# fpthink/3D-WSIS

Measured on AMD Instinct MI355X. Metric: scenes/sec fwd+bwd ScanNet 2cm (~150k voxels) @1/8 GPU; HBM GB/s vs roofline, higher is better.
Workload: dtype f32; 1 GPU; C2: 1 synthetic ScanNet-shaped scene on 1 GPU, 2 cm voxels, fwd+bwd+AdamW step (SubMConv3d UNet 32..160 + ECC GNN + edge affinity + MultiTaskLoss); per-batch segment CSRs / edge graph and all rulebooks are rebuilt inside every step; active_voxels=153685, points=199790, superpoints=2289, edges=20054, scenes_per_gpu=1, global_batch=1, parallelism=scene-sharded dp1

## Files before the change

### 3d-wsis_amd/csrc/loss.hip

```cpp
#include <cstdlib>

#include "common.h"

namespace wsis {
namespace {

constexpr int LOSS_CMAX = 32;
static_assert(LOSS_CMAX == 32, "the error texts of the host checks say 32");
constexpr int SL_THREADS = 256;
constexpr int SL_VALS = 3 * LOSS_CMAX + 2;
constexpr int SL_TP = SL_THREADS + 4;
constexpr int SL_MAX_BLOCKS = 512;

struct SoftmaxRow {
  float v[LOSS_CMAX];
  __device__ __forceinline__ void load(const float* __restrict__ row, int C) {
#pragma unroll
    for (int c = 0; c < LOSS_CMAX; ++c) v[c] = row[c < C ? c : C - 1];
#pragma unroll
    for (int c = 0; c < LOSS_CMAX; ++c) v[c] = c < C ? v[c] : -INFINITY;
  }
  __device__ __forceinline__ float exp_sum(int C, float& Z) {
    float m = v[0];
#pragma unroll
// ... 14 lines not shown
#pragma unroll
  for (int q = 0; q < NV; ++q) {
    double v = (double)a[q];
#pragma unroll
    for (int off = 32; off >= 1; off >>= 1) v += __shfl_xor(v, off, 64);
    if (lane == 0) sh[wave * NV + q] = v;
  }
  __syncthreads();
}
template <int NV, int NW>
__device__ __forceinline__ double block_sum_read(const double* sh, int q) {
  double t = 0.0;
  for (int w = 0; w < NW; ++w) t += sh[w * NV + q];
  return t;
}

__global__ __launch_bounds__(SL_THREADS) void sem_loss_fwd_kernel(const float* __restrict__ x,
                                                                  const int64_t* __restrict__ y, int64_t N, int C,
                                                                  int64_t ignore, float* __restrict__ partial) {
  extern __shared__ __attribute__((aligned(16))) float sl_tile[];
  float A[LOSS_CMAX], B[LOSS_CMAX], K[LOSS_CMAX];
#pragma unroll
  for (int c = 0; c < LOSS_CMAX; ++c) A[c] = B[c] = K[c] = 0.0f;
  float ce = 0.0f, n = 0.0f;
  for (int64_t r = blockIdx.x * (int64_t)blockDim.x + threadIdx.x; r < N; r += (int64_t)gridDim.x * blockDim.x) {
    const int64_t lab = y[r];
    if (lab == ignore) continue;
    SoftmaxRow s;
    s.load(x + r * C, C);
    float xl = 0.0f, Z;
#pragma unroll
    for (int c = 0; c < LOSS_CMAX; ++c)
      if ((int64_t)c == lab && c < C) xl = s.v[c];
    const float m = s.exp_sum(C, Z);
    const float inv = 1.0f / Z, logZ = logf(Z);
#pragma unroll
    for (int c = 0; c < LOSS_CMAX; ++c) {
      const float p = s.v[c] * inv;
      const bool hit = (int64_t)c == lab;
      B[c] += p * p;
      A[c] += hit ? p : 0.0f;
      K[c] += hit ? 1.0f : 0.0f;
    }
    ce += (m + logZ) - xl;
    n += 1.0f;
  }
#pragma unroll
  for (int c = 0; c < LOSS_CMAX; ++c) {
    sl_tile[c * SL_TP + threadIdx.x] = A[c];
    sl_tile[(LOSS_CMAX + c) * SL_TP + threadIdx.x] = B[c];
    sl_tile[(2 * LOSS_CMAX + c) * SL_TP + threadIdx.x] = K[c];
  }
  sl_tile[(3 * LOSS_CMAX) * SL_TP + threadIdx.x] = ce;
  sl_tile[(3 * LOSS_CMAX + 1) * SL_TP + threadIdx.x] = n;
  __syncthreads();
  if (threadIdx.x < SL_VALS) {
    const float4* row = reinterpret_cast<const float4*>(sl_tile + threadIdx.x * SL_TP);
    float s = 0.0f;
#pragma unroll 8
    for (int q = 0; q < SL_THREADS / 4; ++q) {
      const float4 v = row[q];
      s += v.x;
      s += v.y;
      s += v.z;
      s += v.w;
    }
    partial[(int64_t)blockIdx.x * SL_VALS + threadIdx.x] = s;
  }
}

__global__ __launch_bounds__(1024) void sem_loss_final_kernel(const float* __restrict__ partial, int nblk, int C,
                                                              float* __restrict__ out, float* __restrict__ saved) {
  __shared__ double sums[128];
  __shared__ double psub[8][128];
  const int v = threadIdx.x & 127, sub = threadIdx.x >> 7;
  double s = 0.0;
  if (v < SL_VALS)
    for (int b = sub; b < nblk; b += 64) {
      float t[8];
#pragma unroll
      for (int j = 0; j < 8; ++j) {
        const int bb = b + 8 * j;
        t[j] = bb < nblk ? partial[(int64_t)bb * SL_VALS + v] : 0.0f;
      }
#pragma unroll
      for (int j = 0; j < 8; ++j) s += (double)t[j];
    }
  psub[sub][v] = s;
  __syncthreads();
  if (sub == 0)
    sums[v] = ((psub[0][v] + psub[1][v]) + (psub[2][v] + psub[3][v])) + ((psub[4][v] + psub[5][v]) + (psub[6][v] + psub[7][v]));
  __syncthreads();
  if (threadIdx.x == 0) {
    const double eps = 1e-5;
    const double n = sums[3 * LOSS_CMAX + 1];
    double dice_sum = 0.0;
    for (int c = 0; c < C; ++c) {
      const double num = 2.0 * sums[c] + eps;
      const double den = sums[LOSS_CMAX + c] + sums[2 * LOSS_CMAX + c] + 1e-4 + eps;
      saved[c] = (float)num;
      saved[C + c] = (float)den;
      dice_sum += 1.0 - num / den;
    }
    saved[2 * C] = (float)n;
    out[0] = (float)(sums[3 * LOSS_CMAX] / n + dice_sum / (double)C);
    out[1] = (float)n;
  }
}

__global__ __launch_bounds__(SL_THREADS) void sem_loss_bwd_kernel(const float* __restrict__ x,
                                                                  const int64_t* __restrict__ y, int64_t N, int C,
                                                                  int64_t ignore, const float* __restrict__ saved,
                                                                  const float* __restrict__ gout,
                                                                  float* __restrict__ dx) {
  __shared__ float s_num[LOSS_CMAX], s_den[LOSS_CMAX];
  if (threadIdx.x < LOSS_CMAX) {
    s_num[threadIdx.x] = threadIdx.x < C ? saved[threadIdx.x] : 0.0f;
    s_den[threadIdx.x] = threadIdx.x < C ? saved[C + threadIdx.x] : 1.0f;
  }
  __syncthreads();
  const float g = gout[0];
  const float inv_n = 1.0f / saved[2 * C];
  const float inv_c = 1.0f / (float)C;
  __shared__ float tile[SL_THREADS * (LOSS_CMAX + 1)];
  const int pitch = C | 1;
  for (int64_t r0 = blockIdx.x * (int64_t)blockDim.x; r0 < N; r0 += (int64_t)gridDim.x * blockDim.x) {
    const int64_t r = r0 + threadIdx.x;
    float* const mine = tile + threadIdx.x * pitch;
    const int64_t lab = r < N ? y[r] : ignore;
    if (lab == ignore) {
      for (int c = 0; c < C; ++c) mine[c] = 0.0f;
    } else {
      SoftmaxRow s;
      float Z;
      s.load(x + r * C, C);
      s.exp_sum(C, Z);
      const float inv = 1.0f / Z;
      float gp[LOSS_CMAX];
      float dot = 0.0f;
#pragma unroll
      for (int c = 0; c < LOSS_CMAX; ++c) {
        const float p = s.v[c] * inv;
        s.v[c] = p;
        const float den = s_den[c];
        gp[c] = c < C ? inv_c * (2.0f * p * s_num[c] / (den * den) - (((int64_t)c == lab) ? 2.0f / den : 0.0f)) : 0.0f;
        dot += gp[c] * p;
      }
#pragma unroll
      for (int c = 0; c < LOSS_CMAX; ++c)
        if (c < C) mine[c] = g * (s.v[c] * (gp[c] - dot) + (s.v[c] - (((int64_t)c == lab) ? 1.0f : 0.0f)) * inv_n);
    }
    __syncthreads();
    const int64_t rows = N - r0 < (int64_t)blockDim.x ? N - r0 : (int64_t)blockDim.x;
    float* const dst = dx + r0 * C;
    for (int64_t f = threadIdx.x; f < rows * C; f += blockDim.x) {
      const int rr = (int)(f / C), cc = (int)(f - (int64_t)rr * C);
      dst[f] = tile[rr * pitch + cc];
    }
    __syncthreads();
  }
}

constexpr int SR_THREADS = 1024;

struct RegRow {
  float p[3], g[3], np, ip, ig;
  static __device__ __forceinline__ bool dropped(const int64_t* __restrict__ sem, const int64_t* __restrict__ ins,
                                                 int64_t r, int64_t ignore) {
    return sem[r] == ignore || ins[r] == ignore;
  }
  __device__ __forceinline__ void load(const float* __restrict__ p_off, const float* __restrict__ g_off, int64_t r) {
    float pp = 0.f, gg = 0.f;
// ... 187 lines not shown
    const int t = threadIdx.x + u * DL_THREADS;
    v[u] = src[t < n ? t : 0];
  }
}
template <int NU, typename T>
__device__ __forceinline__ void dl_store(const T (&v)[NU], int n, T* dst) {
#pragma unroll
  for (int u = 0; u < NU; ++u) {
    const int t = threadIdx.x + u * DL_THREADS;
    if (t < n) dst[t] = v[u];
  }
}

__device__ __forceinline__ void dl_stage(const float* __restrict__ x, const int64_t* __restrict__ ins,
                                         const int64_t* __restrict__ sem, int S, int I, int64_t ignore, float* xs,
                                         short* slot) {
  constexpr int NR = DL_ROWS / DL_THREADS;
  float v[NR * DL_D];
  int64_t a[NR], b[NR];
  dl_load(x, S * DL_D, v);
  dl_load(ins, S, a);
  dl_load(sem, S, b);
  dl_store(v, S * DL_D, xs);
#pragma unroll
  for (int u = 0; u < NR; ++u) {
    const int r = threadIdx.x + u * DL_THREADS;
    if (r < S) slot[r] = (a[u] != ignore && b[u] != ignore && a[u] >= 0 && a[u] < I) ? (short)a[u] : (short)-1;
  }
}

template <typename On, typename Term>
__device__ __forceinline__ float dl_slot_sums(const short* slot, float* psum, int S, int I, On on, Term term) {
  const int nch = dl_chunks(I), per = I * 8;
  if (threadIdx.x < nch * per) {
    const int ch = threadIdx.x / per, u = threadIdx.x - ch * per;
    const int a = u >> 3, d = u & 7;
    const int r0 = (int)((int64_t)S * ch / nch), r1 = (int)((int64_t)S * (ch + 1) / nch);
    float s = 0.f;
    if (on(a, d)) {
      for (int r = r0; r < r1; r += 8) {
        short sl[8];
        float v[8];
// ... 24 lines not shown
  return fmaxf(2.0f * delta_d - l1, 0.f);
}

__device__ __forceinline__ float dl_mu_norm(const float (*mu)[8], int a) {
  float t2 = 0.f;
#pragma unroll
  for (int d = 0; d < DL_D; ++d) t2 += mu[a][d] * mu[a][d];
  return sqrtf(t2);
}

template <typename T>
__device__ __forceinline__ T dl_pair_den(T n) {
  return n * (n - T(1)) > T(1) ? n * (n - T(1)) : T(1);
}

__global__ __launch_bounds__(DL_THREADS) void disc_loss_fwd_kernel(const float* __restrict__ x,
                                                                   const int64_t* __restrict__ ins,
                                                                   const int64_t* __restrict__ sem, int S, int I,
                                                                   int64_t ignore, DlParams P, float* __restrict__ out,
                                                                   float* __restrict__ saved) {
  __shared__ float xs[DL_ROWS * DL_D];
  __shared__ short slot[DL_ROWS];
  __shared__ float mu[DL_SLOTS][8];
  __shared__ float psum[DL_THREADS];
  __shared__ double red[DL_THREADS / 64];
  dl_stage(x, ins, sem, S, I, ignore, xs, slot);
  __syncthreads();
  const float sum = dl_slot_sums(slot, psum, S, I, [](int, int) { return true; },
                                 [&](int, int d, int r) { return d < DL_D ? xs[r * DL_D + d] : 1.0f; });
  if (threadIdx.x < I * 8) mu[threadIdx.x >> 3][threadIdx.x & 7] = sum;
  __syncthreads();
  {
    const bool act = threadIdx.x < I * 8;
    const int a = threadIdx.x >> 3, d = threadIdx.x & 7;
    const float c = act ? mu[a][7] : 1.0f, sv = act ? mu[a][d] : 0.0f;
    __syncthreads();
    if (act && d < DL_D) mu[a][d] = sv / fmaxf(c, 1.0f);
  }
  __syncthreads();
  double lvar = 0.0, ldist = 0.0, lreg = 0.0, n = 0.0;
  float* kk = saved + DL_SLOTS * 8;
  for (int r = threadIdx.x; r < S; r += DL_THREADS) {
    const int a = slot[r];
    float k = 0.f;
    if (a >= 0) {
      float t2 = 0.f;
#pragma unroll
      for (int d = 0; d < DL_D; ++d) {
        const float e = xs[r * DL_D + d] - mu[a][d];
        t2 += e * e;
      }
      const float t = sqrtf(t2), h = fmaxf(t - P.delta_v, 0.f);
      lvar += (double)(h * h / mu[a][7]);
      k = t > 0.f ? 2.0f * h / t : 0.f;
    }
    kk[r] = k;
  }
  for (int q = threadIdx.x; q < I * I; q += DL_THREADS) {
    const int a = q / I, b = q - a * I;
    if (a != b && mu[a][7] > 0.f && mu[b][7] > 0.f) {
      const float h = dl_pair_hinge(mu, a, b, P.delta_d);
      ldist += (double)(h * h);
    }
  }
  if (threadIdx.x < I && mu[threadIdx.x][7] > 0.f) {
    lreg = (double)dl_mu_norm(mu, threadIdx.x);
    n = 1.0;
  }
  auto total = [&](double v) {
    const double one[1] = {v};
    __syncthreads();
    block_sum_stage(one, red);
    return block_sum_read<1, DL_THREADS / 64>(red, 0);
  };
  lvar = total(lvar), ldist = total(ldist), lreg = total(lreg), n = total(n);
  for (int t = threadIdx.x; t < DL_SLOTS * 8; t += DL_THREADS) saved[t] = (t >> 3) < I ? mu[t >> 3][t & 7] : 0.f;
  if (threadIdx.x == 0) {
    out[0] = (float)(P.p_var * (lvar / n) + P.p_dist * (ldist / dl_pair_den(n)) + P.p_reg * lreg);
    saved[DL_SLOTS * 8 + DL_ROWS] = (float)n;
  }
}

__global__ __launch_bounds__(DL_THREADS) void disc_loss_bwd_kernel(const float* __restrict__ x,
                                                                   const int64_t* __restrict__ ins,
                                                                   const int64_t* __restrict__ sem, int S, int I,
                                                                   int64_t ignore, DlParams P,
                                                                   const float* __restrict__ saved,
                                                                   const float* __restrict__ gout,
                                                                   float* __restrict__ dx) {
  __shared__ float xs[DL_ROWS * DL_D];
  __shared__ short slot[DL_ROWS];
  __shared__ float mu[DL_SLOTS][8];
  __shared__ float gmu[DL_SLOTS][8];
  __shared__ float psum[DL_THREADS];
  __shared__ float kk[DL_ROWS];
  dl_stage(x, ins, sem, S, I, ignore, xs, slot);
  for (int t = threadIdx.x; t < DL_SLOTS * 8; t += DL_THREADS) mu[t >> 3][t & 7] = saved[t];
  {
    float kv[DL_ROWS / DL_THREADS];
    dl_load(saved + DL_SLOTS * 8, S, kv);
    dl_store(kv, S, kk);
  }
  __syncthreads();
  const float n = saved[DL_SLOTS * 8 + DL_ROWS];
  const float den = dl_pair_den(n);
  const float via = dl_slot_sums(slot, psum, S, I, [&](int a, int d) { return d < DL_D && mu[a][7] > 0.f; },
                                 [&](int a, int d, int r) { return kk[r] * (xs[r * DL_D + d] - mu[a][d]); });
  if (threadIdx.x < I * 8) {
    const int a = threadIdx.x >> 3, d = threadIdx.x & 7;
    float gsum = 0.f;
    const float c = mu[a][7];
    if (d < DL_D && c > 0.f) {
      for (int b = 0; b < I; ++b) {
        if (b == a || !(mu[b][7] > 0.f)) continue;
        const float h = dl_pair_hinge(mu, a, b, P.delta_d);
        const float df = mu[a][d] - mu[b][d];
        const float sg = df > 0.f ? 1.f : (df < 0.f ? -1.f : 0.f);
        gsum += (P.p_dist / den) * 4.0f * h * (-sg);
      }
      const float nm = dl_mu_norm(mu, a);
      if (nm > 0.f) gsum += P.p_reg * mu[a][d] / nm;
      gsum += -(P.p_var / (n * c)) * via;
    }
    gmu[a][d] = gsum;
  }
  __syncthreads();
  const float g = gout[0];
  for (int t = threadIdx.x; t < S * DL_D; t += DL_THREADS) {
    const int r = t / DL_D, d = t - r * DL_D;
    const int a = slot[r];
    float v = 0.f;
    if (a >= 0) {
      const float c = mu[a][7];
      v = g * ((P.p_var / (n * c)) * kk[r] * (xs[t] - mu[a][d]) + gmu[a][d] / c);
    }
    dx[t] = v;
  }
}

const char* disc_loss_bad_args(const float* x, const int64_t* ins, const int64_t* sem, int64_t S, int32_t D,
                               int32_t n_slots, const float* saved) {
  if (!(S >= 1 && S <= DL_ROWS && D == DL_D && n_slots >= 1 && n_slots <= DL_SLOTS))
    return "1 <= rows <= 4096, 7 features, 1 <= slots <= 64";
  return x && ins && sem && saved ? nullptr : "null pointer";
}

int sl_blocks(int64_t N) {
  const char* e = tune_env("WSIS_SL_BLOCKS");
  int cap = e ? atoi(e) : 256;
  if (cap < 1 || cap > SL_MAX_BLOCKS) cap = SL_MAX_BLOCKS;
  int64_t b = ceil_div(N > 0 ? N : 1, SL_THREADS);
  if (b > cap) b = cap;
  return (int)b;
}

}
}

using namespace wsis;
// ... 8 lines not shown
int wsis_semantic_loss_fwd(const float* d_scores, const int64_t* d_labels, int64_t N, int32_t C, int64_t ignore_label,
                           float* d_out2, float* d_saved, void* d_ws, int64_t ws_bytes, void* stream) {
  WSIS_REQUIRE(N >= 0 && C >= 1 && C <= LOSS_CMAX, "1 <= classes <= 32");
  WSIS_REQUIRE(d_out2 && d_saved && d_ws, "null pointer");
  WSIS_REQUIRE(N == 0 || (d_scores && d_labels), "null input");
  WSIS_REQUIRE(ws_bytes >= wsis_semantic_loss_workspace_bytes(N), "workspace too small");
  hipStream_t st = as_stream(stream);
  const int nblk = sl_blocks(N);
  float* partial = static_cast<float*>(d_ws);
  const size_t ldsb = (size_t)SL_VALS * SL_TP * sizeof(float);
  static bool attr_set = false;
  if (!attr_set) {
    WSIS_HIP_CHECK(hipFuncSetAttribute((const void*)sem_loss_fwd_kernel, hipFuncAttributeMaxDynamicSharedMemorySize, (int)ldsb));
    attr_set = true;
  }
  hipLaunchKernelGGL(sem_loss_fwd_kernel, dim3(nblk), dim3(SL_THREADS), ldsb, st, d_scores, d_labels, N, (int)C,
                     ignore_label, partial);
  WSIS_LAUNCH_CHECK();
  hipLaunchKernelGGL(sem_loss_final_kernel, dim3(1), dim3(1024), 0, st, partial, nblk, (int)C, d_out2, d_saved);
  WSIS_LAUNCH_CHECK();
  return WSIS_OK;
}

int wsis_semantic_loss_bwd(const float* d_scores, const int64_t* d_labels, int64_t N, int32_t C, int64_t ignore_label,
                           const float* d_saved, const float* d_grad_loss, float* d_dscores, void* stream) {
  WSIS_REQUIRE(N >= 0 && C >= 1 && C <= LOSS_CMAX, "1 <= classes <= 32");
  if (N == 0) return WSIS_OK;
  WSIS_REQUIRE(d_scores && d_labels && d_saved && d_grad_loss && d_dscores, "null pointer");
  hipLaunchKernelGGL(sem_loss_bwd_kernel, dim3(grid_for(N, SL_THREADS)), dim3(SL_THREADS), 0, as_stream(stream),
                     d_scores, d_labels, N, (int)C, ignore_label, d_saved, d_grad_loss, d_dscores);
  WSIS_LAUNCH_CHECK();
  return WSIS_OK;
}

int wsis_sp_regression_loss_fwd(const float* d_pred_off, const float* d_gt_off, const float* d_pred_occ,
                                const float* d_gt_occ, const float* d_pred_size, const float* d_gt_size,
                                const int64_t* d_sem_label, const int64_t* d_ins_label, int64_t S,
                                int64_t ignore_label, float* d_out5, void* stream) {
  WSIS_REQUIRE(S >= 0 && d_out5, "bad args");
  WSIS_REQUIRE(S == 0 || (d_pred_off && d_gt_off && d_pred_occ && d_gt_occ && d_pred_size && d_gt_size &&
                          d_sem_label && d_ins_label), "null pointer");
  hipLaunchKernelGGL(sp_reg_fwd_kernel, dim3(1), dim3(SR_THREADS), 0, as_stream(stream), d_pred_off, d_gt_off,
                     d_pred_occ, d_gt_occ, d_pred_size, d_gt_size, d_sem_label, d_ins_label, S, ignore_label, d_out5);
  WSIS_LAUNCH_CHECK();
  return WSIS_OK;
// ... 56 lines not shown
  hipLaunchKernelGGL(loss_sum_kernel, dim3(1), dim3(1), 0, as_stream(stream), t[0], t[1], t[2], t[3], t[4], t[5], t[6], t[7], (int)n,
                     (unsigned)paired, d_out);
  WSIS_LAUNCH_CHECK();
  return WSIS_OK;
}

int32_t wsis_disc_loss_saved_floats(void) { return DL_SLOTS * 8 + DL_ROWS + 1; }

int wsis_disc_loss_fwd(const float* d_x, const int64_t* d_ins_label, const int64_t* d_sem_label, int64_t S,
                       int32_t D, int32_t n_slots, int64_t ignore_label, float delta_v, float delta_d, float p_var,
                       float p_dist, float p_reg, float* d_out1, float* d_saved, void* stream) {
  const char* bad = disc_loss_bad_args(d_x, d_ins_label, d_sem_label, S, D, n_slots, d_saved);
  WSIS_REQUIRE(!bad, bad);
  WSIS_REQUIRE(d_out1, "null pointer");
  const DlParams P = {delta_v, delta_d, p_var, p_dist, p_reg};
  hipLaunchKernelGGL(disc_loss_fwd_kernel, dim3(1), dim3(DL_THREADS), 0, as_stream(stream), d_x, d_ins_label,
                     d_sem_label, (int)S, (int)n_slots, ignore_label, P, d_out1, d_saved);
  WSIS_LAUNCH_CHECK();
  return WSIS_OK;
}

int wsis_disc_loss_bwd(const float* d_x, const int64_t* d_ins_label, const int64_t* d_sem_label, int64_t S,
                       int32_t D, int32_t n_slots, int64_t ignore_label, float delta_v, float delta_d, float p_var,
                       float p_dist, float p_reg, const float* d_saved, const float* d_grad_loss, float* d_dx,
                       void* stream) {
  const char* bad = disc_loss_bad_args(d_x, d_ins_label, d_sem_label, S, D, n_slots, d_saved);
  WSIS_REQUIRE(!bad, bad);
  WSIS_REQUIRE(d_grad_loss && d_dx, "null pointer");
  const DlParams P = {delta_v, delta_d, p_var, p_dist, p_reg};
  hipLaunchKernelGGL(disc_loss_bwd_kernel, dim3(1), dim3(DL_THREADS), 0, as_stream(stream), d_x, d_ins_label,
                     d_sem_label, (int)S, (int)n_slots, ignore_label, P, d_saved, d_grad_loss, d_dx);
  WSIS_LAUNCH_CHECK();
  return WSIS_OK;
}

}
```

### 3d-wsis_amd/model/losses_3D_WSIS.py

```python
import functools
import os

import torch
import torch.nn as nn
import torch.nn.functional as F


class _NullLogger(object):
    def info(self, *a, **k):
        pass


def _ops():
    import wsis_ops
    return wsis_ops


def _on(switch, default="1"):
    return os.environ.get(switch, default) != "0"


class MultiTaskLoss(nn.Module):
    def __init__(self, logger, param_loss, param_model):
        super().__init__()
# ... 126 lines not shown
    def _sp_discriminative(self, inp, indexed, valid, loss_out):
        feats, sp_batch_offsets = inp["sp_discriminative_features"]
        sp_sem_labels, sp_ins_labels = inp["superpoint_labels"]
        offs = [int(o) for o in sp_batch_offsets]
        slots = inp.get("sp_instance_slots")
        d_losses = []
        for i in range(1, len(offs)):
            b, e = offs[i - 1], offs[i]
            n_slots = int(slots[i - 1]) if slots is not None else 0
            ins = sp_ins_labels[b:e]
            if indexed:
                keep = valid()[0][b:e]
                d_loss, _, _, _ = self.discriminative_loss(feats[b:e][keep], ins[keep])
            elif (feats.is_cuda and self.discriminative_feature_dim == 7 and _on("WSIS_FUSE_DISC_LOSS")
                  and 1 <= n_slots <= _ops().DISC_MAX_SLOTS and 1 <= e - b <= _ops().DISC_MAX_ROWS):
                d_loss = _ops().discriminative_loss(feats[b:e], ins, sp_sem_labels[b:e], n_slots, self.ignore_label,
                                                    self.delta_v, self.delta_d, self.param_var, self.param_dist,
                                                    self.param_reg)
            elif 1 <= n_slots <= 512:
                d_loss = self.discriminative_loss_slots(feats[b:e], ins, valid()[0][b:e], n_slots)
            else:
                d_loss = self.discriminative_loss_masked(feats[b:e], ins, valid()[0][b:e])
            d_losses.append(d_loss.view(-1))
        sp_d_loss = torch.mean(torch.cat(d_losses)) if len(d_losses) != 1 else d_losses[0].reshape(())
        loss_out["superpoint_discriminative_loss"] = (sp_d_loss, feats.shape[0])
        return sp_d_loss

    def _sum_terms(self, terms, paired):
        for name, t in terms:
            self._log(name, t)
        terms = [t for _, t in terms]
# ... 98 lines not shown
```

### 3d-wsis_amd/wsis_ops.py

```python
import ctypes
import os

import numpy as np
import torch
from torch.autograd import Function

import wsis_native as _n
from torch_scatter import SegmentCSR


def branch_stream(device, i=0):
    if os.environ.get("WSIS_BRANCH", "1") == "0" or device.type != "cuda":
        return None
    from spconv import ops as sp_ops
    return sp_ops._side_stream(device)


class EdgeGraph(object):

    def __init__(self, edge_u, edge_v, num_nodes, num_src=None, csr_u=None, csr_v=None):
        _n.require_cuda(edge_u, edge_v)
        self.eu = edge_u.contiguous().long()
        self.ev = edge_v.contiguous().long()
        self.E = self.eu.numel()
# ... 835 lines not shown
        lib = _n.hip()
        scores = scores.contiguous().float()
        labels = labels.contiguous().long()
        N, C = scores.shape
        out = torch.empty(2, dtype=torch.float32, device=scores.device)
        saved = torch.empty(2 * C + 1, dtype=torch.float32, device=scores.device)
        ws_bytes = lib.wsis_semantic_loss_workspace_bytes(N)
        ws = torch.empty(ws_bytes, dtype=torch.uint8, device=scores.device)
        _n.check(lib.wsis_semantic_loss_fwd(_n.ptr(scores), _n.ptr(labels), N, C, int(ignore_label), _n.ptr(out),
                                            _n.ptr(saved), _n.ptr(ws), ws_bytes, _n.stream_ptr()),
                 "semantic_loss_fwd")
        ctx.save_for_backward(scores, labels, saved)
        ctx.ignore_label = int(ignore_label)
        loss, n_valid = out[0], out[1]
        ctx.mark_non_differentiable(n_valid)
        return loss, n_valid

    @staticmethod
    def backward(ctx, g_loss, _g_n):
        scores, labels, saved = ctx.saved_tensors
        N, C = scores.shape
        d = torch.empty_like(scores)
        g = g_loss.contiguous().float()
        _n.check(_n.hip().wsis_semantic_loss_bwd(_n.ptr(scores), _n.ptr(labels), N, C, ctx.ignore_label,
                                                 _n.ptr(saved), _n.ptr(g), _n.ptr(d), _n.stream_ptr()),
                 "semantic_loss_bwd")
        return d, None, None


def semantic_point_loss(scores, labels, ignore_label=-100):
    return _SemanticPointLoss.apply(scores, labels, ignore_label)


class _SpCrossEntropy(Function):

# ... 1 lines not shown
    def forward(ctx, scores, labels, ignore_label):
        _n.require_cuda(scores, labels)
        scores = scores.contiguous().float()
        labels = labels.contiguous().long()
        S, C = scores.shape
        out = torch.empty(3, dtype=torch.float32, device=scores.device)
        lib = _n.hip()
        ws_bytes = lib.wsis_sp_ce_loss_workspace_bytes(S)
        ws = torch.empty(ws_bytes, dtype=torch.uint8, device=scores.device)
        _n.check(lib.wsis_sp_ce_loss_fwd(_n.ptr(scores), _n.ptr(labels), S, C, int(ignore_label), _n.ptr(out), _n.ptr(ws),
                                         ws_bytes, _n.ptr(_n.sync_block(scores.device)), _n.stream_ptr()), "sp_ce_loss_fwd")
        ctx.save_for_backward(scores, labels, out)
        ctx.ignore_label = int(ignore_label)
        loss, total = out[0], out[1]
        ctx.mark_non_differentiable(total)
        return loss, total

    @staticmethod
    def backward(ctx, g_loss, _g_total):
        scores, labels, out = ctx.saved_tensors
        S, C = scores.shape
        d = torch.empty_like(scores)
        _n.check(_n.hip().wsis_sp_ce_loss_bwd(_n.ptr(scores), _n.ptr(labels), S, C, ctx.ignore_label, _n.ptr(out),
                                              _n.ptr(g_loss.contiguous().float()), _n.ptr(d), _n.stream_ptr()),
                 "sp_ce_loss_bwd")
        return d, None, None


def superpoint_cross_entropy(scores, labels, ignore_label=-100):
    return _SpCrossEntropy.apply(scores, labels, ignore_label)


class _LossSum(Function):

    @staticmethod
# ... 24 lines not shown
        pred_off, gt_off, pred_occ, gt_occ, pred_size, gt_size = (f(pred_off), f(gt_off), f(pred_occ), f(gt_occ),
                                                                  f(pred_size), f(gt_size))
        sem_label, ins_label = sem_label.contiguous().long(), ins_label.contiguous().long()
        S = pred_off.shape[0]
        assert pred_off.shape == (S, 3) and gt_off.shape == (S, 3) and pred_occ.numel() == S and pred_size.numel() == S
        out = torch.empty(5, dtype=torch.float32, device=pred_off.device)
        _n.check(_n.hip().wsis_sp_regression_loss_fwd(
            _n.ptr(pred_off), _n.ptr(gt_off), _n.ptr(pred_occ), _n.ptr(gt_occ), _n.ptr(pred_size), _n.ptr(gt_size),
            _n.ptr(sem_label), _n.ptr(ins_label), S, int(ignore_label), _n.ptr(out), _n.stream_ptr()),
            "sp_regression_loss_fwd")
        ctx.save_for_backward(pred_off, gt_off, pred_occ, gt_occ, pred_size, gt_size, sem_label, ins_label, out)
        ctx.ignore_label = int(ignore_label)
        ctx.shapes = (pred_occ.shape, pred_size.shape)
        n_valid = out[4]
        ctx.mark_non_differentiable(n_valid)
        return out[0], out[1], out[2], out[3], n_valid

    @staticmethod
    def backward(ctx, g_norm, g_dir, g_occ, g_size, _g_n):
        pred_off, gt_off, pred_occ, gt_occ, pred_size, gt_size, sem_label, ins_label, out = ctx.saved_tensors
        S = pred_off.shape[0]
        d_off = torch.empty_like(pred_off)
        d_occ = torch.empty_like(pred_occ)
        d_size = torch.empty_like(pred_size)
        g = [t.contiguous().float() for t in (g_norm, g_dir, g_occ, g_size)]
        _n.check(_n.hip().wsis_sp_regression_loss_bwd(
            _n.ptr(pred_off), _n.ptr(gt_off), _n.ptr(pred_occ), _n.ptr(gt_occ), _n.ptr(pred_size), _n.ptr(gt_size),
            _n.ptr(sem_label), _n.ptr(ins_label), S, ctx.ignore_label, _n.ptr(out), _n.ptr(g[0]), _n.ptr(g[1]),
            _n.ptr(g[2]), _n.ptr(g[3]), _n.ptr(d_off), _n.ptr(d_occ), _n.ptr(d_size), _n.stream_ptr()),
            "sp_regression_loss_bwd")
        return d_off, None, d_occ, None, d_size, None, None, None, None


def sp_regression_losses(pred_off, gt_off, pred_occ, gt_occ, pred_size, gt_size, sem_label, ins_label,
                         ignore_label=-100):
    return _SpRegressionLoss.apply(pred_off, gt_off, pred_occ, gt_occ, pred_size, gt_size, sem_label, ins_label,
                                   ignore_label)


LOSS_MAX_CLASSES, LOSS_SUM_MAX_TERMS = 32, 8
# ... 36 lines not shown
```

Before: 135.5 scenes/s.

## Add tiled coalesced semantic-loss backward, sorted disc-loss kernels, and skip null grads

Adds a semantic-loss backward kernel that stages each block's 256 score rows into LDS with float4 coalesced loads and writes dx back with float4 stores, replacing per-thread strided row loads. Adds sorted-segment discriminative-loss forward and backward kernels that count rows per slot and reduce by segment. Widens the final reduction's loads per iteration, and makes the autograd functions skip backward work when no gradient arrives. All of this is selected by a new env plan flag that defaults on. The cost is more shared memory per block and more code paths to keep correct.

```diff
diff --git a/3d-wsis_amd/csrc/loss.hip b/3d-wsis_amd/csrc/loss.hip
--- a/3d-wsis_amd/csrc/loss.hip
+++ b/3d-wsis_amd/csrc/loss.hip
@@ -52,6 +52,87 @@
   for (int w = 0; w < NW; ++w) t += sh[w * NV + q];
   return t;
 }
+
+constexpr int SL_NQ = LOSS_CMAX / 4;
+constexpr int SL_ROWTILE = SL_THREADS * (LOSS_CMAX + 1);
+struct RowTrip {
+  float4 q[SL_NQ];
+  const float* src;
+  int nf;
+  bool pieces;
+  __device__ __forceinline__ void load(const float* __restrict__ x, int64_t r0, int64_t N, int C) {
+    src = x + r0 * C;
+    const int rows = N - r0 < (int64_t)SL_THREADS ? (int)(N - r0) : SL_THREADS;
+    const int npiece = SL_THREADS / 4 * C;
+    nf = rows * C;
+    pieces = rows == SL_THREADS && (reinterpret_cast<uintptr_t>(x) & 15) == 0;
+    if (pieces) {
+#pragma unroll
+      for (int u = 0; u < SL_NQ; ++u)
+        if (u * SL_THREADS < npiece) {
+          const int i = threadIdx.x + u * SL_THREADS;
+          q[u] = reinterpret_cast<const float4*>(src)[i < npiece ? i : npiece - 1];
+        }
+    }
+  }
+  __device__ __forceinline__ void store(float* tile, int C) const {
+    const int pitch = C | 1, npiece = SL_THREADS / 4 * C;
+    const float inv_c = 1.0f / (float)C;
+    if (pieces) {
+#pragma unroll
+      for (int u = 0; u < SL_NQ; ++u) {
+        const int i = threadIdx.x + u * SL_THREADS;
+        if (u * SL_THREADS < npiece && i < npiece) {
+          int f = 4 * i;
+          asm volatile("" : "+v"(f));
+          int row = (int)(((float)f + 0.5f) * inv_c);
+          int col = f - row * C;
+          const float e[4] = {q[u].x, q[u].y, q[u].z, q[u].w};
+#pragma unroll
+          for (int k = 0; k < 4; ++k) {
+            tile[row * pitch + col] = e[k];
+            if (++col == C) col = 0, ++row;
+          }
+        }
+      }
+    } else {
+      for (int f = threadIdx.x; f < nf; f += SL_THREADS) {
+        const int row = (int)(((float)f + 0.5f) * inv_c);
+        tile[row * pitch + (f - row * C)] = src[f];
+      }
+    }
+  }
+};
+
+__device__ __forceinline__ int trip_row(int pitch) {
+  int o = threadIdx.x * pitch;
+  asm volatile("" : "+v"(o));
+  return o;
+}
+
+__device__ __forceinline__ void sem_fwd_row(SoftmaxRow& s, int64_t lab, int C, float (&A)[LOSS_CMAX],
+                                            float (&B)[LOSS_CMAX], float (&K)[LOSS_CMAX], float& ce, float& n) {
+  float xl = 0.0f, Z;
+#pragma unroll
+  for (int c = 0; c < LOSS_CMAX; ++c)
+    if ((int64_t)c == lab && c < C) xl = s.v[c];
+  const float m = s.exp_sum(C, Z);
+  const float inv = 1.0f / Z, logZ = logf(Z);
+#pragma unroll
+  for (int c = 0; c < LOSS_CMAX; ++c) {
+    const float p = s.v[c] * inv;
+    const bool hit = (int64_t)c == lab;
+    B[c] += p * p;
+    A[c] += hit ? p : 0.0f;
+    K[c] += hit ? 1.0f : 0.0f;
+  }
+  ce += (m + logZ) - xl;
+  n += 1.0f;
+}
+
+__device__ __forceinline__ void sem_fwd_reduce(float* sl_tile, const float (&A)[LOSS_CMAX], const float (&B)[LOSS_CMAX],
+                                               const float (&K)[LOSS_CMAX], float ce, float n,
+                                               float* __restrict__ partial);
 
 __global__ __launch_bounds__(SL_THREADS) void sem_loss_fwd_kernel(const float* __restrict__ x,
                                                                   const int64_t* __restrict__ y, int64_t N, int C,
@@ -66,23 +147,14 @@
     if (lab == ignore) continue;
     SoftmaxRow s;
     s.load(x + r * C, C);
-    float xl = 0.0f, Z;
-#pragma unroll
-    for (int c = 0; c < LOSS_CMAX; ++c)
-      if ((int64_t)c == lab && c < C) xl = s.v[c];
-    const float m = s.exp_sum(C, Z);
-    const float inv = 1.0f / Z, logZ = logf(Z);
-#pragma unroll
-    for (int c = 0; c < LOSS_CMAX; ++c) {
-      const float p = s.v[c] * inv;
-      const bool hit = (int64_t)c == lab;
-      B[c] += p * p;
-      A[c] += hit ? p : 0.0f;
-      K[c] += hit ? 1.0f : 0.0f;
-    }
-    ce += (m + logZ) - xl;
-    n += 1.0f;
-  }
+    sem_fwd_row(s, lab, C, A, B, K, ce, n);
+  }
+  sem_fwd_reduce(sl_tile, A, B, K, ce, n, partial);
+}
+
+__device__ __forceinline__ void sem_fwd_reduce(float* sl_tile, const float (&A)[LOSS_CMAX], const float (&B)[LOSS_CMAX],
+                                               const float (&K)[LOSS_CMAX], float ce, float n,
+                                               float* __restrict__ partial) {
 #pragma unroll
   for (int c = 0; c < LOSS_CMAX; ++c) {
     sl_tile[c * SL_TP + threadIdx.x] = A[c];
@@ -107,6 +179,7 @@
   }
 }
 
+template <int NL>
 __global__ __launch_bounds__(1024) void sem_loss_final_kernel(const float* __restrict__ partial, int nblk, int C,
                                                               float* __restrict__ out, float* __restrict__ saved) {
   __shared__ double sums[128];
@@ -114,15 +187,18 @@
   const int v = threadIdx.x & 127, sub = threadIdx.x >> 7;
   double s = 0.0;
   if (v < SL_VALS)
-    for (int b = sub; b < nblk; b += 64) {
-      float t[8];
-#pragma unroll
-      for (int j = 0; j < 8; ++j) {
+    for (int b = sub; b < nblk; b += 8 * NL) {
+      float t[NL];
+#pragma unroll
+      for (int j = 0; j < NL; ++j) {
         const int bb = b + 8 * j;
-        t[j] = bb < nblk ? partial[(int64_t)bb * SL_VALS + v] : 0.0f;
+        if (NL == 8)
+          t[j] = bb < nblk ? partial[(int64_t)bb * SL_VALS + v] : 0.0f;
+        else
+          t[j] = partial[(int64_t)(bb < nblk ? bb : nblk - 1) * SL_VALS + v];
       }
 #pragma unroll
-      for (int j = 0; j < 8; ++j) s += (double)t[j];
+      for (int j = 0; j < NL; ++j) s += b + 8 * j < nblk ? (double)t[j] : 0.0;
     }
   psub[sub][v] = s;
   __syncthreads();
@@ -144,6 +220,26 @@
     out[0] = (float)(sums[3 * LOSS_CMAX] / n + dice_sum / (double)C);
     out[1] = (float)n;
   }
+}
+
+__device__ __forceinline__ void sem_bwd_row(SoftmaxRow& s, int64_t lab, int C, const float* s_num, const float* s_den,
+                                            float g, float inv_n, float inv_c, float* mine) {
+  float Z;
+  s.exp_sum(C, Z);
+  const float inv = 1.0f / Z;
+  float gp[LOSS_CMAX];
+  float dot = 0.0f;
+#pragma unroll
+  for (int c = 0; c < LOSS_CMAX; ++c) {
+    const float p = s.v[c] * inv;
+    s.v[c] = p;
+    const float den = s_den[c];
+    gp[c] = c < C ? inv_c * (2.0f * p * s_num[c] / (den * den) - (((int64_t)c == lab) ? 2.0f / den : 0.0f)) : 0.0f;
+    dot += gp[c] * p;
+  }
+#pragma unroll
+  for (int c = 0; c < LOSS_CMAX; ++c)
+    if (c < C) mine[c] = g * (s.v[c] * (gp[c] - dot) + (s.v[c] - (((int64_t)c == lab) ? 1.0f : 0.0f)) * inv_n);
 }
 
 __global__ __launch_bounds__(SL_THREADS) void sem_loss_bwd_kernel(const float* __restrict__ x,
@@ -170,23 +266,8 @@
       for (int c = 0; c < C; ++c) mine[c] = 0.0f;
     } else {
       SoftmaxRow s;
-      float Z;
       s.load(x + r * C, C);
-      s.exp_sum(C, Z);
-      const float inv = 1.0f / Z;
-      float gp[LOSS_CMAX];
-      float dot = 0.0f;
-#pragma unroll
-      for (int c = 0; c < LOSS_CMAX; ++c) {
-        const float p = s.v[c] * inv;
-        s.v[c] = p;
-        const float den = s_den[c];
-        gp[c] = c < C ? inv_c * (2.0f * p * s_num[c] / (den * den) - (((int64_t)c == lab) ? 2.0f / den : 0.0f)) : 0.0f;
-        dot += gp[c] * p;
-      }
-#pragma unroll
-      for (int c = 0; c < LOSS_CMAX; ++c)
-        if (c < C) mine[c] = g * (s.v[c] * (gp[c] - dot) + (s.v[c] - (((int64_t)c == lab) ? 1.0f : 0.0f)) * inv_n);
+      sem_bwd_row(s, lab, C, s_num, s_den, g, inv_n, inv_c, mine);
     }
     __syncthreads();
     const int64_t rows = N - r0 < (int64_t)blockDim.x ? N - r0 : (int64_t)blockDim.x;
@@ -194,6 +275,63 @@
     for (int64_t f = threadIdx.x; f < rows * C; f += blockDim.x) {
       const int rr = (int)(f / C), cc = (int)(f - (int64_t)rr * C);
       dst[f] = tile[rr * pitch + cc];
+    }
+    __syncthreads();
+  }
+}
+
+__global__ __launch_bounds__(SL_THREADS, 3) void sem_loss_bwd_tiled_kernel(const float* __restrict__ x,
+                                                                        const int64_t* __restrict__ y, int64_t N,
+                                                                        int C, int64_t ignore,
+                                                                        const float* __restrict__ saved,
+                                                                        const float* __restrict__ gout,
+                                                                        float* __restrict__ dx) {
+  __shared__ float s_num[LOSS_CMAX], s_den[LOSS_CMAX];
+  __shared__ __attribute__((aligned(16))) float tile[SL_ROWTILE];
+  if (threadIdx.x < LOSS_CMAX) {
+    s_num[threadIdx.x] = threadIdx.x < C ? saved[threadIdx.x] : 0.0f;
+    s_den[threadIdx.x] = threadIdx.x < C ? saved[C + threadIdx.x] : 1.0f;
+  }
+  const float g = gout[0];
+  const float inv_n = 1.0f / saved[2 * C];
+  const float inv_c = 1.0f / (float)C;
+  const int pitch = C | 1;
+  const bool vec = (reinterpret_cast<uintptr_t>(dx) & 15) == 0;
+  for (int64_t r0 = blockIdx.x * (int64_t)SL_THREADS; r0 < N; r0 += (int64_t)gridDim.x * SL_THREADS) {
+    const int64_t r = r0 + threadIdx.x;
+    const int64_t lab = r < N ? y[r] : ignore;
+    RowTrip trip;
+    trip.load(x, r0, N, C);
+    trip.store(tile, C);
+    __syncthreads();
+    float* const mine = tile + trip_row(pitch);
+    if (lab == ignore) {
+      for (int c = 0; c < C; ++c) mine[c] = 0.0f;
+    } else {
+      SoftmaxRow s;
+      s.load(mine, C);
+      sem_bwd_row(s, lab, C, s_num, s_den, g, inv_n, inv_c, mine);
+    }
+    __syncthreads();
+    const int rows = N - r0 < (int64_t)SL_THREADS ? (int)(N - r0) : SL_THREADS;
+    const int nf = rows * C;
+    float* const dst = dx + r0 * C;
+    for (int f = 4 * threadIdx.x; f < nf; f += 4 * SL_THREADS) {
+      int row = (int)(((float)f + 0.5f) * inv_c);
+      int col = f - row * C;
+      float e[4];
+#pragma unroll
+      for (int k = 0; k < 4; ++k) {
+        e[k] = f + k < nf ? tile[row * pitch + col] : 0.0f;
+        if (++col == C) col = 0, ++row;
+      }
+      if (vec && f + 3 < nf) {
+        *reinterpret_cast<float4*>(dst + f) = make_float4(e[0], e[1], e[2], e[3]);
+      } else {
+#pragma unroll
+        for (int k = 0; k < 4; ++k)
+          if (f + k < nf) dst[f + k] = e[k];
+      }
     }
     __syncthreads();
   }
@@ -411,18 +549,26 @@
 
 __device__ __forceinline__ void dl_stage(const float* __restrict__ x, const int64_t* __restrict__ ins,
                                          const int64_t* __restrict__ sem, int S, int I, int64_t ignore, float* xs,
-                                         short* slot) {
+                                         short* slot, int* cnt = nullptr) {
   constexpr int NR = DL_ROWS / DL_THREADS;
   float v[NR * DL_D];
   int64_t a[NR], b[NR];
   dl_load(x, S * DL_D, v);
   dl_load(ins, S, a);
   dl_load(sem, S, b);
+  if (cnt) {
+    if (threadIdx.x < DL_SLOTS) cnt[threadIdx.x] = 0;
+    __syncthreads();
+  }
   dl_store(v, S * DL_D, xs);
 #pragma unroll
   for (int u = 0; u < NR; ++u) {
     const int r = threadIdx.x + u * DL_THREADS;
-    if (r < S) slot[r] = (a[u] != ignore && b[u] != ignore && a[u] >= 0 && a[u] < I) ? (short)a[u] : (short)-1;
+    if (r < S) {
+      const short sl = (a[u] != ignore && b[u] != ignore && a[u] >= 0 && a[u] < I) ? (short)a[u] : (short)-1;
+      slot[r] = sl;
+      if (cnt && sl >= 0) atomicAdd(&cnt[sl], 1);
+    }
   }
 }
 
@@ -477,6 +623,86 @@
   return n * (n - T(1)) > T(1) ? n * (n - T(1)) : T(1);
 }
 
+__device__ __forceinline__ void dl_fwd_terms(const float* xs, const short* slot, const float (*mu)[8], int S, int I,
+                                             const DlParams& P, float* __restrict__ saved, double (&t4)[4]) {
+  t4[0] = t4[1] = t4[2] = t4[3] = 0.0;
+  float* kk = saved + DL_SLOTS * 8;
+  for (int r = threadIdx.x; r < S; r += DL_THREADS) {
+    const int a = slot[r];
+    float k = 0.f;
+    if (a >= 0) {
+      float t2 = 0.f;
+#pragma unroll
+      for (int d = 0; d < DL_D; ++d) {
+        const float e = xs[r * DL_D + d] - mu[a][d];
+        t2 += e * e;
+      }
+      const float t = sqrtf(t2), h = fmaxf(t - P.delta_v, 0.f);
+      t4[0] += (double)(h * h / mu[a][7]);
+      k = t > 0.f ? 2.0f * h / t : 0.f;
+    }
+    kk[r] = k;
+  }
+  for (int q = threadIdx.x; q < I * I; q += DL_THREADS) {
+    const int a = q / I, b = q - a * I;
+    if (a != b && mu[a][7] > 0.f && mu[b][7] > 0.f) {
+      const float h = dl_pair_hinge(mu, a, b, P.delta_d);
+      t4[1] += (double)(h * h);
+    }
+  }
+  if (threadIdx.x < I && mu[threadIdx.x][7] > 0.f) {
+    t4[2] = (double)dl_mu_norm(mu, threadIdx.x);
+    t4[3] = 1.0;
+  }
+}
+
+__device__ __forceinline__ void dl_fwd_finish(const float (*mu)[8], int I, const DlParams& P, const double (&tot)[4],
+                                              float* __restrict__ out, float* __restrict__ saved) {
+  for (int t = threadIdx.x; t < DL_SLOTS * 8; t += DL_THREADS) saved[t] = (t >> 3) < I ? mu[t >> 3][t & 7] : 0.f;
+  if (threadIdx.x == 0) {
+    const double n = tot[3];
+    out[0] = (float)(P.p_var * (tot[0] / n) + P.p_dist * (tot[1] / dl_pair_den(n)) + P.p_reg * tot[2]);
+    saved[DL_SLOTS * 8 + DL_ROWS] = (float)n;
+  }
+}
+
+__device__ __forceinline__ void dl_bwd_gmu(const float (*mu)[8], float (*gmu)[8], float via, int I, const DlParams& P,
+                                           float n, float den) {
+  if (threadIdx.x < I * 8) {
+    const int a = threadIdx.x >> 3, d = threadIdx.x & 7;
+    float gsum = 0.f;
+    const float c = mu[a][7];
+    if (d < DL_D && c > 0.f) {
+      for (int b = 0; b < I; ++b) {
+        if (b == a || !(mu[b][7] > 0.f)) continue;
+        const float h = dl_pair_hinge(mu, a, b, P.delta_d);
+        const float df = mu[a][d] - mu[b][d];
+        const float sg = df > 0.f ? 1.f : (df < 0.f ? -1.f : 0.f);
+        gsum += (P.p_dist / den) * 4.0f * h * (-sg);
+      }
+      const float nm = dl_mu_norm(mu, a);
+      if (nm > 0.f) gsum += P.p_reg * mu[a][d] / nm;
+      gsum += -(P.p_var / (n * c)) * via;
+    }
+    gmu[a][d] = gsum;
+  }
+}
+
+__device__ __forceinline__ void dl_bwd_dx(const float* xs, const short* slot, const float* kk, const float (*mu)[8],
+                                          const float (*gmu)[8], int S, const DlParams& P, float n, float g,
+                                          float* __restrict__ dx) {
+  for (int t = threadIdx.x; t < S * DL_D; t += DL_THREADS) {
+    const int r = t / DL_D, d = t - r * DL_D;
+    const int a = slot[r];
+    float v = 0.f;
+    if (a >= 0) {
+      const float c = mu[a][7];
+      v = g * ((P.p_var / (n * c)) * kk[r] * (xs[t] - mu[a][d]) + gmu[a][d] / c);
+    }
+    dx[t] = v;
+  }
+}
+
 __global__ __launch_bounds__(DL_THREADS) void disc_loss_fwd_kernel(const float* __restrict__ x,
                                                                    const int64_t* __restrict__ ins,
                                                                    const int64_t* __restrict__ sem, int S, int I,
@@ -501,47 +727,17 @@
     if (act && d < DL_D) mu[a][d] = sv / fmaxf(c, 1.0f);
   }
   __syncthreads();
-  double lvar = 0.0, ldist = 0.0, lreg = 0.0, n = 0.0;
-  float* kk = saved + DL_SLOTS * 8;
-  for (int r = threadIdx.x; r < S; r += DL_THREADS) {
-    const int a = slot[r];
-    float k = 0.f;
-    if (a >= 0) {
-      float t2 = 0.f;
-#pragma unroll
-      for (int d = 0; d < DL_D; ++d) {
-        const float e = xs[r * DL_D + d] - mu[a][d];
-        t2 += e * e;
-      }
-      const float t = sqrtf(t2), h = fmaxf(t - P.delta_v, 0.f);
-      lvar += (double)(h * h / mu[a][7]);
-      k = t > 0.f ? 2.0f * h / t : 0.f;
-    }
-    kk[r] = k;
-  }
-  for (int q = threadIdx.x; q < I * I; q += DL_THREADS) {
-    const int a = q / I, b = q - a * I;
-    if (a != b && mu[a][7] > 0.f && mu[b][7] > 0.f) {
-      const float h = dl_pair_hinge(mu, a, b, P.delta_d);
-      ldist += (double)(h * h);
-    }
-  }
-  if (threadIdx.x < I && mu[threadIdx.x][7] > 0.f) {
-    lreg = (double)dl_mu_norm(mu, threadIdx.x);
-    n = 1.0;
-  }
+  double t4[4];
+  dl_fwd_terms(xs, slot, mu, S, I, P, saved, t4);
   auto total = [&](double v) {
     const double one[1] = {v};
     __syncthreads();
     block_sum_stage(one, red);
     return block_sum_read<1, DL_THREADS / 64>(red, 0);
   };
-  lvar = total(lvar), ldist = total(ldist), lreg = total(lreg), n = total(n);
-  for (int t = threadIdx.x; t < DL_SLOTS * 8; t += DL_THREADS) saved[t] = (t >> 3) < I ? mu[t >> 3][t & 7] : 0.f;
-  if (threadIdx.x == 0) {
-    out[0] = (float)(P.p_var * (lvar / n) + P.p_dist * (ldist / dl_pair_den(n)) + P.p_reg * lreg);
-    saved[DL_SLOTS * 8 + DL_ROWS] = (float)n;
-  }
+#pragma unroll
+  for (int q = 0; q < 4; ++q) t4[q] = total(t4[q]);
+  dl_fwd_finish(mu, I, P, t4, out, saved);
 }
 
 __global__ __launch_bounds__(DL_THREADS) void disc_loss_bwd_kernel(const float* __restrict__ x,
@@ -569,36 +765,155 @@
   const float den = dl_pair_den(n);
   const float via = dl_slot_sums(slot, psum, S, I, [&](int a, int d) { return d < DL_D && mu[a][7] > 0.f; },
                                  [&](int a, int d, int r) { return kk[r] * (xs[r * DL_D + d] - mu[a][d]); });
-  if (threadIdx.x < I * 8) {
-    const int a = threadIdx.x >> 3, d = threadIdx.x & 7;
-    float gsum = 0.f;
-    const float c = mu[a][7];
-    if (d < DL_D && c > 0.f) {
-      for (int b = 0; b < I; ++b) {
-        if (b == a || !(mu[b][7] > 0.f)) continue;
-        const float h = dl_pair_hinge(mu, a, b, P.delta_d);
-        const float df = mu[a][d] - mu[b][d];
-        const float sg = df > 0.f ? 1.f : (df < 0.f ? -1.f : 0.f);
-        gsum += (P.p_dist / den) * 4.0f * h * (-sg);
+  dl_bwd_gmu(mu, gmu, via, I, P, n, den);
+  __syncthreads();
+  dl_bwd_dx(xs, slot, kk, mu, gmu, S, P, n, gout[0], dx);
+}
+
+static_assert(DL_SLOTS == 64 && DL_THREADS / 64 * 4 == DL_SLOTS, "one lane per slot in the scan, four slots per wave");
+constexpr int DL_WSLOTS = 4;
+
+struct DlSegments {
+  int off[DL_WSLOTS], num[DL_WSLOTS];
+  __device__ __forceinline__ void sort(const short* slot, const int* cnt, short* list, int S) {
+    const int lane = threadIdx.x & 63, wave = threadIdx.x >> 6;
+    const int c = cnt[lane];
+    int inc = c;
+#pragma unroll
+    for (int d = 1; d < 64; d <<= 1) {
+      const int o = __shfl_up(inc, d, 64);
+      if (lane >= d) inc += o;
+    }
+    int base[DL_WSLOTS];
+#pragma unroll
+    for (int k = 0; k < DL_WSLOTS; ++k) {
+      off[k] = base[k] = __shfl(inc - c, wave + 16 * k, 64);
+      num[k] = __shfl(c, wave + 16 * k, 64);
+    }
+    const unsigned long long below = (1ull << lane) - 1ull;
+    for (int r0 = 0; r0 < S; r0 += 256) {
+      int s[4];
+#pragma unroll
+      for (int u = 0; u < 4; ++u) {
+        const int r = r0 + 64 * u + lane;
+        s[u] = r < S ? (int)slot[r] : -1;
       }
-      const float nm = dl_mu_norm(mu, a);
-      if (nm > 0.f) gsum += P.p_reg * mu[a][d] / nm;
-      gsum += -(P.p_var / (n * c)) * via;
-    }
-    gmu[a][d] = gsum;
-  }
-  __syncthreads();
-  const float g = gout[0];
-  for (int t = threadIdx.x; t < S * DL_D; t += DL_THREADS) {
-    const int r = t / DL_D, d = t - r * DL_D;
-    const int a = slot[r];
-    float v = 0.f;
-    if (a >= 0) {
-      const float c = mu[a][7];
-      v = g * ((P.p_var / (n * c)) * kk[r] * (xs[t] - mu[a][d]) + gmu[a][d] / c);
-    }
-    dx[t] = v;
-  }
+#pragma unroll
+      for (int u = 0; u < 4; ++u)
+#pragma unroll
+        for (int k = 0; k < DL_WSLOTS; ++k) {
+          const bool hit = s[u] == wave + 16 * k;
+          const unsigned long long m = __ballot(hit);
+          if (hit) list[base[k] + __popcll(m & below)] = (short)(r0 + 64 * u + lane);
+          base[k] += __popcll(m);
+        }
+    }
+  }
+  template <typename Term>
+  __device__ __forceinline__ float sum(const short* list, int k, Term term) const {
+    const int lane = threadIdx.x & 63, j = lane >> 3, d = lane & 7;
+    const int o = off[k], n = num[k];
+    float s = 0.f;
+    for (int i = j; i < n; i += 32) {
+      float v[4];
+#pragma unroll
+      for (int u = 0; u < 4; ++u) {
+        const int ii = i + 8 * u < n ? i + 8 * u : n - 1;
+        v[u] = term(d, (int)list[o + ii]);
+      }
+#pragma unroll
+      for (int u = 0; u < 4; ++u)
+        if (i + 8 * u < n) s += v[u];
+    }
+#pragma unroll
+    for (int x = 8; x < 64; x <<= 1) s += __shfl_xor(s, x, 64);
+    return s;
+  }
+};
+
+__global__ __launch_bounds__(DL_THREADS) void disc_loss_fwd_sorted_kernel(const float* __restrict__ x,
+                                                                          const int64_t* __restrict__ ins,
+                                                                          const int64_t* __restrict__ sem, int S, int I,
+                                                                          int64_t ignore, DlParams P,
+                                                                          float* __restrict__ out,
+                                                                          float* __restrict__ saved) {
+  __shared__ float xs[DL_ROWS * DL_D];
+  __shared__ short slot[DL_ROWS];
+  __shared__ short list[DL_ROWS];
+  __shared__ int cnt[DL_SLOTS];
+  __shared__ float mu[DL_SLOTS][8];
+  __shared__ double red[DL_THREADS / 64 * 4];
+  dl_stage(x, ins, sem, S, I, ignore, xs, slot, cnt);
+  __syncthreads();
+  DlSegments seg;
+  seg.sort(slot, cnt, list, S);
+  __syncthreads();
+  {
+    const int lane = threadIdx.x & 63, wave = threadIdx.x >> 6;
+#pragma unroll
+    for (int k = 0; k < DL_WSLOTS; ++k) {
+      const int a = wave + 16 * k;
+      if (a >= I) break;
+      const float sum = seg.sum(list, k, [&](int d, int r) { return d < DL_D ? xs[r * DL_D + d] : 0.0f; });
+      const float c = (float)seg.num[k];
+      if (lane < 8) mu[a][lane] = lane < DL_D ? sum / fmaxf(c, 1.0f) : c;
+    }
+  }
+  __syncthreads();
+  double t4[4];
+  dl_fwd_terms(xs, slot, mu, S, I, P, saved, t4);
+  block_sum_stage(t4, red);
+#pragma unroll
+  for (int q = 0; q < 4; ++q) t4[q] = block_sum_read<4, DL_THREADS / 64>(red, q);
+  dl_fwd_finish(mu, I, P, t4, out, saved);
+}
+
+__global__ __launch_bounds__(DL_THREADS) void disc_loss_bwd_sorted_kernel(const float* __restrict__ x,
+                                                                          const int64_t* __restrict__ ins,
+                                                                          const int64_t* __restrict__ sem, int S, int I,
+                                                                          int64_t ignore, DlParams P,
+                                                                          const float* __restrict__ saved,
+                                                                          const float* __restrict__ gout,
+                                                                          float* __restrict__ dx) {
+  __shared__ float xs[DL_ROWS * DL_D];
+  __shared__ short slot[DL_ROWS];
+  __shared__ short list[DL_ROWS];
+  __shared__ int cnt[DL_SLOTS];
+  __shared__ float mu[DL_SLOTS][8];
+  __shared__ float gmu[DL_SLOTS][8];
+  __shared__ float vs[DL_SLOTS][8];
+  __shared__ float kk[DL_ROWS];
+  dl_stage(x, ins, sem, S, I, ignore, xs, slot, cnt);
+  for (int t = threadIdx.x; t < DL_SLOTS * 8; t += DL_THREADS) mu[t >> 3][t & 7] = saved[t];
+  {
+    float kv[DL_ROWS / DL_THREADS];
+    dl_load(saved + DL_SLOTS * 8, S, kv);
+    dl_store(kv, S, kk);
+  }
+  __syncthreads();
+  const float n = saved[DL_SLOTS * 8 + DL_ROWS];
+  const float den = dl_pair_den(n);
+  DlSegments seg;
+  seg.sort(slot, cnt, list, S);
+  __syncthreads();
+  {
+    const int lane = threadIdx.x & 63, wave = threadIdx.x >> 6;
+#pragma unroll
+    for (int k = 0; k < DL_WSLOTS; ++k) {
+      const int a = wave + 16 * k;
+      if (a >= I) break;
+      float via = 0.f;
+      if (mu[a][7] > 0.f) {
+        const float m = mu[a][lane & 7];
+        via = seg.sum(list, k, [&](int d, int r) { return d < DL_D ? kk[r] * (xs[r * DL_D + d] - m) : 0.0f; });
+      }
+      if (lane < 8) vs[a][lane] = via;
+    }
+  }
+  __syncthreads();
+  dl_bwd_gmu(mu, gmu, threadIdx.x < I * 8 ? vs[threadIdx.x >> 3][threadIdx.x & 7] : 0.f, I, P, n, den);
+  __syncthreads();
+  dl_bwd_dx(xs, slot, kk, mu, gmu, S, P, n, gout[0], dx);
 }
 
 const char* disc_loss_bad_args(const float* x, const int64_t* ins, const int64_t* sem, int64_t S, int32_t D,
@@ -606,6 +921,11 @@
   if (!(S >= 1 && S <= DL_ROWS && D == DL_D && n_slots >= 1 && n_slots <= DL_SLOTS))
     return "1 <= rows <= 4096, 7 features, 1 <= slots <= 64";
   return x && ins && sem && saved ? nullptr : "null pointer";
+}
+
+int loss_plan() {
+  const char* e = getenv("WSIS_LOSS_PLAN");
+  return e ? atoi(e) : 1;
 }
 
 int sl_blocks(int64_t N) {
@@ -644,10 +964,11 @@
     WSIS_HIP_CHECK(hipFuncSetAttribute((const void*)sem_loss_fwd_kernel, hipFuncAttributeMaxDynamicSharedMemorySize, (int)ldsb));
     attr_set = true;
   }
+  const auto fin = loss_plan() != 0 ? sem_loss_final_kernel<32> : sem_loss_final_kernel<8>;
   hipLaunchKernelGGL(sem_loss_fwd_kernel, dim3(nblk), dim3(SL_THREADS), ldsb, st, d_scores, d_labels, N, (int)C,
                      ignore_label, partial);
   WSIS_LAUNCH_CHECK();
-  hipLaunchKernelGGL(sem_loss_final_kernel, dim3(1), dim3(1024), 0, st, partial, nblk, (int)C, d_out2, d_saved);
+  hipLaunchKernelGGL(fin, dim3(1), dim3(1024), 0, st, partial, nblk, (int)C, d_out2, d_saved);
   WSIS_LAUNCH_CHECK();
   return WSIS_OK;
 }
@@ -657,8 +978,9 @@
   WSIS_REQUIRE(N >= 0 && C >= 1 && C <= LOSS_CMAX, "1 <= classes <= 32");
   if (N == 0) return WSIS_OK;
   WSIS_REQUIRE(d_scores && d_labels && d_saved && d_grad_loss && d_dscores, "null pointer");
-  hipLaunchKernelGGL(sem_loss_bwd_kernel, dim3(grid_for(N, SL_THREADS)), dim3(SL_THREADS), 0, as_stream(stream),
-                     d_scores, d_labels, N, (int)C, ignore_label, d_saved, d_grad_loss, d_dscores);
+  const auto bwd = loss_plan() != 0 ? sem_loss_bwd_tiled_kernel : sem_loss_bwd_kernel;
+  hipLaunchKernelGGL(bwd, dim3(grid_for(N, SL_THREADS)), dim3(SL_THREADS), 0, as_stream(stream), d_scores, d_labels, N,
+                     (int)C, ignore_label, d_saved, d_grad_loss, d_dscores);
   WSIS_LAUNCH_CHECK();
   return WSIS_OK;
 }
@@ -745,8 +1067,9 @@
   WSIS_REQUIRE(!bad, bad);
   WSIS_REQUIRE(d_out1, "null pointer");
   const DlParams P = {delta_v, delta_d, p_var, p_dist, p_reg};
-  hipLaunchKernelGGL(disc_loss_fwd_kernel, dim3(1), dim3(DL_THREADS), 0, as_stream(stream), d_x, d_ins_label,
-                     d_sem_label, (int)S, (int)n_slots, ignore_label, P, d_out1, d_saved);
+  const auto fwd = loss_plan() != 0 ? disc_loss_fwd_sorted_kernel : disc_loss_fwd_kernel;
+  hipLaunchKernelGGL(fwd, dim3(1), dim3(DL_THREADS), 0, as_stream(stream), d_x, d_ins_label, d_sem_label, (int)S,
+                     (int)n_slots, ignore_label, P, d_out1, d_saved);
   WSIS_LAUNCH_CHECK();
   return WSIS_OK;
 }
@@ -759,8 +1082,9 @@
   WSIS_REQUIRE(!bad, bad);
   WSIS_REQUIRE(d_grad_loss && d_dx, "null pointer");
   const DlParams P = {delta_v, delta_d, p_var, p_dist, p_reg};
-  hipLaunchKernelGGL(disc_loss_bwd_kernel, dim3(1), dim3(DL_THREADS), 0, as_stream(stream), d_x, d_ins_label,
-                     d_sem_label, (int)S, (int)n_slots, ignore_label, P, d_saved, d_grad_loss, d_dx);
+  const auto bwd = loss_plan() != 0 ? disc_loss_bwd_sorted_kernel : disc_loss_bwd_kernel;
+  hipLaunchKernelGGL(bwd, dim3(1), dim3(DL_THREADS), 0, as_stream(stream), d_x, d_ins_label, d_sem_label, (int)S,
+                     (int)n_slots, ignore_label, P, d_saved, d_grad_loss, d_dx);
   WSIS_LAUNCH_CHECK();
   return WSIS_OK;
 }
diff --git a/3d-wsis_amd/model/losses_3D_WSIS.py b/3d-wsis_amd/model/losses_3D_WSIS.py
--- a/3d-wsis_amd/model/losses_3D_WSIS.py
+++ b/3d-wsis_amd/model/losses_3D_WSIS.py
@@ -164,7 +164,8 @@
                 d_loss, _, _, _ = self.discriminative_loss(feats[b:e][keep], ins[keep])
             elif (feats.is_cuda and self.discriminative_feature_dim == 7 and _on("WSIS_FUSE_DISC_LOSS")
                   and 1 <= n_slots <= _ops().DISC_MAX_SLOTS and 1 <= e - b <= _ops().DISC_MAX_ROWS):
-                d_loss = _ops().discriminative_loss(feats[b:e], ins, sp_sem_labels[b:e], n_slots, self.ignore_label,
+                x = feats if (b == 0 and e == feats.shape[0]) else feats[b:e]
+                d_loss = _ops().discriminative_loss(x, ins, sp_sem_labels[b:e], n_slots, self.ignore_label,
                                                     self.delta_v, self.delta_d, self.param_var, self.param_dist,
                                                     self.param_reg)
             elif 1 <= n_slots <= 512:
diff --git a/3d-wsis_amd/wsis_ops.py b/3d-wsis_amd/wsis_ops.py
--- a/3d-wsis_amd/wsis_ops.py
+++ b/3d-wsis_amd/wsis_ops.py
@@ -873,11 +873,14 @@
         ctx.ignore_label = int(ignore_label)
         loss, n_valid = out[0], out[1]
         ctx.mark_non_differentiable(n_valid)
+        ctx.set_materialize_grads(False)
         return loss, n_valid
 
     @staticmethod
     def backward(ctx, g_loss, _g_n):
         scores, labels, saved = ctx.saved_tensors
+        if g_loss is None:
+            return None, None, None
         N, C = scores.shape
         d = torch.empty_like(scores)
         g = g_loss.contiguous().float()
@@ -909,11 +912,14 @@
         ctx.ignore_label = int(ignore_label)
         loss, total = out[0], out[1]
         ctx.mark_non_differentiable(total)
+        ctx.set_materialize_grads(False)
         return loss, total
 
     @staticmethod
     def backward(ctx, g_loss, _g_total):
         scores, labels, out = ctx.saved_tensors
+        if g_loss is None:
+            return None, None, None
         S, C = scores.shape
         d = torch.empty_like(scores)
         _n.check(_n.hip().wsis_sp_ce_loss_bwd(_n.ptr(scores), _n.ptr(labels), S, C, ctx.ignore_label, _n.ptr(out),
@@ -968,6 +974,7 @@
         ctx.shapes = (pred_occ.shape, pred_size.shape)
         n_valid = out[4]
         ctx.mark_non_differentiable(n_valid)
+        ctx.set_materialize_grads(False)
         return out[0], out[1], out[2], out[3], n_valid
 
     @staticmethod
@@ -977,7 +984,15 @@
         d_off = torch.empty_like(pred_off)
         d_occ = torch.empty_like(pred_occ)
         d_size = torch.empty_like(pred_size)
-        g = [t.contiguous().float() for t in (g_norm, g_dir, g_occ, g_size)]
+        if g_norm is None and g_dir is None and g_occ is None and g_size is None:
+            return (None,) * 9
+        zero = None
+        g = []
+        for t in (g_norm, g_dir, g_occ, g_size):
+            if t is None:
+                zero = torch.zeros((), dtype=torch.float32, device=out.device) if zero is None else zero
+                t = zero
+            g.append(t.contiguous().float())
         _n.check(_n.hip().wsis_sp_regression_loss_bwd(
             _n.ptr(pred_off), _n.ptr(gt_off), _n.ptr(pred_occ), _n.ptr(gt_occ), _n.ptr(pred_size), _n.ptr(gt_size),
             _n.ptr(sem_label), _n.ptr(ins_label), S, ctx.ignore_label, _n.ptr(out), _n.ptr(g[0]), _n.ptr(g[1]),
```

After: 135.5 scenes/s. Within noise of the previous version (-0.0%).
